# zuds-survey/zuds-pipeline

Measured on AMD Instinct MI355X. Metric: Mpix/s resample->coadd->subtract, 3072x3072 frames, higher is better.
Workload: dtype f32; 1 GPU; configs[1]+[2]: 32x 3072x3072 TPV frames/GPU, mesh background + weight rescale + Lanczos-3 resample + WEIGHTED coadd (+ AND mask coadd, int16 masks); then 1 science frame/GPU: align ref, hotpants 3x3 regions x 10x10 stamps, r=10, ko=4, subtract; frames_per_gpu=32, size=3072, mask_dtype=int16, combine=WEIGHTED, subtract=True

## Files before the change

zuds-pipeline_amd/csrc/hotpants.hip:

```cpp
#include "hp_dev.h"
#include <sched.h>
#include "chol_diag.h"

__global__ void k_hp_valid(const float* __restrict__ sci, const float* __restrict__ ref,
                           const uint8_t* __restrict__ bpm, int64_t n, float il, float iu,
                           float tl, float tu, uint8_t* __restrict__ bad,
                           const double* __restrict__ lim, double nsig) {
    int64_t p = (int64_t)blockIdx.x * blockDim.x + threadIdx.x;
    if (lim) {
        il = (float)(lim[0] - nsig * lim[1]);
        tl = (float)(lim[3] - nsig * lim[4]);
    }
    if (p >= n) return;
    float s = sci[p], t = ref[p];
    bool ok = (s == s) && (t == t) && fabsf(s) < 3e38f && fabsf(t) < 3e38f;
    ok = ok && s >= il && s <= iu && t >= tl && t <= tu;
    if (bpm) ok = ok && bpm[p] == 0;
    bad[p] = ok ? 0 : 1;
}

#define HP_ROWMAX 16384
__global__ __launch_bounds__(256) void k_hp_rowany(const uint8_t* __restrict__ in, int nx, int ny, int hw,
                                                   uint8_t* __restrict__ out) {
    extern __shared__ int ra_pre[];
// ... 2258 lines not shown
    hp_merit_body(P, G, phi, vbar, active, xsol, merit, guard, needlist);
}
__global__ __launch_bounds__(64) void k_hp_merit_b(const hp_plan P, const hp_job* __restrict__ jobs, int round) {
    const hp_job& J = jobs[blockIdx.z];
    hp_merit_body(P, J.G, J.phi, J.vbar, J.active, J.rhs, J.merit, HPJ_GUARD(J, round), J.needlist);
}

__global__ __launch_bounds__(64) void k_hp_reject_wave(const hp_plan P, const double* __restrict__ merit,
                                                       const int2* __restrict__ centres, int* __restrict__ active,
                                                       int* __restrict__ need, int* __restrict__ chg,
                                                       int* __restrict__ nrej, double* __restrict__ stats,
                                                       const int* __restrict__ guard, int* __restrict__ round_flag,
                                                       int* __restrict__ needlist, const int* __restrict__ tmo,
                                                       const hp_sig sig) {
    hp_reject_wave_body(P, merit, centres, active, need, chg, nrej, stats, guard, round_flag, needlist, tmo);
    hp_round_signal(sig, round_flag, gridDim.x);
}
__global__ __launch_bounds__(64) void k_hp_reject_wave_b(const hp_plan P, const hp_job* __restrict__ jobs, int round) {
    const hp_job& J = jobs[blockIdx.z];
    hp_reject_wave_body(P, J.merit, J.centres, J.active, J.need, J.chg, HPJ_NREJ(J), J.stats, HPJ_GUARD(J, round),
                        J.rflags + round, J.needlist);
}

__global__ void k_hp_flag(int32_t* __restrict__ mask, const float* __restrict__ img, float value, int32_t bit,
                          int64_t n, const int* __restrict__ tmo, int nreg) {
    int gaveup = 0;
    for (int r = 0; r < nreg; ++r) gaveup |= tmo[r];
    if (gaveup) return;
    int64_t p = (int64_t)blockIdx.x * blockDim.x + threadIdx.x;
    if (p >= n) return;
    if (img[p] == value) mask[p] |= bit;
}

extern "C" void zm_hp_params_default(zm_hp_params* p) {
    if (!p) return;
    memset(p, 0, sizeof(*p));
    p->tu = 5e3; p->tl = 0.0; p->iu = 5e3; p->il = 0.0;
    p->r = 10.0; p->rss = 15.0;
    p->fin = sqrt(50000.0); p->fi = 1e-30;
    p->nsx = p->nsy = 10; p->nrx = p->nry = 1;
    p->ko = 4; p->bgo = 0; p->nss = 3; p->normalize = 0;
    p->ft = 20.0; p->ks = 2.0;
    p->ngauss = 3;
    p->deg[0] = 6; p->deg[1] = 4; p->deg[2] = 2;
    p->sigma[0] = 0.7; p->sigma[1] = 1.5; p->sigma[2] = 3.0;
    p->limits_dev = nullptr; p->limits_nsigma = 10.0;
}

static int make_plan(const zm_hp_params* hp, int nx, int ny, hp_plan* P, std::vector<double>* filt,
                     std::vector<double>* basis) {
    memset(P, 0, sizeof(*P));
    P->nx = nx; P->ny = ny;
    P->hwk = (int)hp->r; P->hwss = (int)hp->rss;
    ZM_CHECK(P->hwk >= 1 && P->hwk <= HP_MAX_HWK, "zm_subtract: kernel half width int(r) = %d outside [1, %d]", P->hwk, HP_MAX_HWK);
    ZM_CHECK(P->hwss >= 1 && P->hwss <= HP_MAX_HWSS, "zm_subtract: substamp half width int(rss) = %d outside [1, %d]", P->hwss, HP_MAX_HWSS);
    P->hw = P->hwk + P->hwss;
    P->step = 2 * P->hwk + 1; P->sw = 2 * P->hwss + 1; P->pw = 2 * P->hw + 1;
    P->npix = P->sw * P->sw;
    P->npixp = (P->npix + GR_KT - 1) / GR_KT * GR_KT;
    ZM_CHECK(hp->ngauss >= 1 && hp->ngauss <= 4, "zm_subtract: ngauss %d outside [1, 4]", hp->ngauss);
    ZM_CHECK(hp->ko >= 0 && hp->ko <= 6, "zm_subtract: -ko %d outside [0, 6]", hp->ko);
    ZM_CHECK(hp->bgo >= 0 && hp->bgo <= 3, "zm_subtract: -bgo %d outside [0, 3]", hp->bgo);
    ZM_CHECK(hp->nss >= 1 && hp->nss <= HP_MAXNSS, "zm_subtract: nss %d outside [1, %d]", hp->nss, HP_MAXNSS);
    ZM_CHECK(hp->nrx >= 1 && hp->nry >= 1 && hp->nrx * hp->nry <= HP_MAXREG, "zm_subtract: bad -nrx/-nry");
    ZM_CHECK(hp->nsx >= 1 && hp->nsy >= 1 && hp->nsx * hp->nsy <= 4096, "zm_subtract: bad -nsx/-nsy");
    P->ko = hp->ko; P->bgo = hp->bgo; P->nss = hp->nss; P->normalize = hp->normalize;
// ... 288 lines not shown
    const int* h_int = reinterpret_cast<const int*>(h_sum);
    const double* h_stats = reinterpret_cast<const double*>(h_sum + sizeof(int) * HP_NIBUF);
    const double* h_x0 = h_stats + 2 * HP_MAXREG;
    int rounds = 0, retries = 0, ntimeouts = 0;
    const char* spin_env = getenv("ZM_CHOL_SPIN_LIMIT");
    hp_fit_guard fitting(&g_hp_fitting[ctx->device & 63]);
    for (int attempt = 0; attempt < 2; ++attempt) {
    const bool safe = attempt > 0;
    const int spin_limit = (!safe && spin_env) ? atoi(spin_env) : CF_SPIN_LIMIT;
    ZM_HIP(hipMemsetAsync(ibuf, 0, sizeof(int) * HP_NIBUF, st));
    ZM_TRY(hp_launch_cells(ctx, P, ref, bad, dirty, centres, active, need, ntotal));
    const hv_cfg hvc = hp_vectors_cfg(P.pw, P.sw, P.npix);
    ZM_CHECK(hvc.cw >= 8, "zm_subtract: r = %d, rss = %d: the template patch alone exceeds the LDS", P.hwk, P.hwss);
    size_t vsh = hvc.shmem;
    const int hv_gx = hvc.big ? std::min(P.ncell, 128) : P.ncell;
    double* hv_w0g = nullptr;
    if (hvc.w0_global)
        ZM_TRY(ctx->get("hp_w0g", sizeof(double) * (size_t)hv_gx * HV_SPLIT_FEW * P.npix, (void**)&hv_w0g));

    int* rflags = nullptr;
    int* h_rflags = nullptr;
    hipEvent_t* evs = nullptr;
    ZM_TRY(ctx->get("hp_rflags", sizeof(int) * 32, (void**)&rflags));
    ZM_TRY(ctx->get_pinned("hp_rflags_h", sizeof(int) * 16, (void**)&h_rflags));
    ZM_TRY(zm_get_sync_events(ctx, 3, &evs));
    ZM_HIP(hipMemsetAsync(rflags, 0, sizeof(int) * 32, st));
    if (!ctx->hp_sig_h) {
        ZM_HIP(hipHostMalloc((void**)&ctx->hp_sig_h, sizeof(unsigned long long) * 16, hipHostMallocCoherent | hipHostMallocMapped));
        memset(ctx->hp_sig_h, 0, sizeof(unsigned long long) * 16);
        ZM_HIP(hipHostGetDevicePointer((void**)&ctx->hp_sig_d, ctx->hp_sig_h, 0));
    }
    static const bool sig_off = ZM_DEVENV("ZM_HP_SIGNAL") && ZM_DEVENV("ZM_HP_SIGNAL")[0] == '0';
    const unsigned seq = ++ctx->hp_seq;
    auto enqueue_round = [&](const int rounds) -> int {
        const int* guard = rounds > 1 ? rflags + (rounds - 1) : nullptr;
        const int ncl_grid = std::min(P.ncell, 48);
        if (rounds > 1) {
            zm_scope_timer t(ctx, "hp_solve");
            int nt = zm_div_up(P.nunk, 16);
            if (P.nkp > 16)
                hipLaunchKernelGGL(k_hp_build, dim3(nt, nt, P.nreg), b256, 0, st, P, G, phi, active, chg, -1, A0, rhs0, guard);
        }
        {
            zm_scope_timer t(ctx, "hp_vectors");
            ZM_TRY(zm_hp_launch_vectors(ctx, st, P, hvc, rounds, ncl_grid, hv_gx, sci, ref, sci_rms, ref_rms, d_filt, centres, active,
                                        need, X, phi, vbar, guard, phiold, needlist, hv_w0g));
            ZM_HIP(hipGetLastError());
        }
        {
            zm_scope_timer t(ctx, "hp_gram");
            hipLaunchKernelGGL(k_hp_gram, dim3(rounds == 1 ? P.ncell : ncl_grid, GR_SPLIT), b256, 0, st, P, X, need, active, Gp, guard,
                               rounds == 1 ? nullptr : needlist);
            hipLaunchKernelGGL(k_hp_gram_sum, dim3(rounds == 1 ? P.ncell : ncl_grid), dim3(GS_THREADS), 0, st, Gp, need, active, G, guard, Gold,
                               rounds == 1 ? nullptr : needlist);
            ZM_HIP(hipGetLastError());
        }
        {
            zm_scope_timer t(ctx, "hp_solve");
            int nt = zm_div_up(P.nunk, 16);
            const char* form_env = getenv("ZM_CHOL_FORM");
            bool tp = safe || ctx->share >= 2 || fitting.shared();
            if (form_env && !strcmp(form_env, "tp")) tp = true;
            if (form_env && (!strcmp(form_env, "lat") || !strcmp(form_env, "df")) && !safe) tp = false;
            if (!ctx->hp_wg_cap) {
                int occ = 0, ncu = 0;
                ZM_HIP(hipOccupancyMaxActiveBlocksPerMultiprocessor(&occ, (const void*)k_chol_fused, 256, 0));
                ZM_HIP(hipDeviceGetAttribute(&ncu, hipDeviceAttributeMultiprocessorCount, ctx->device));
                ctx->hp_wg_cap = std::max(1, std::min(occ, 1) * (ncu - ncu / 16));
                if (ZM_DEVENV("ZM_CHOL_PROF")) fprintf(stderr, "chol: occupancy %d x %d CUs\n", occ, ncu);
            }
            const int wg_cap = ctx->hp_wg_cap / std::max(ctx->share, 1);
            const int W = std::max(2, std::min(68, wg_cap / P.nreg));
            const int nunk = P.nunk;
            static const bool want_prof = ZM_DEVENV("ZM_CHOL_PROF") && atoi(ZM_DEVENV("ZM_CHOL_PROF")) != 0;
            const bool want_df = !tp && !(form_env && !strcmp(form_env, "lat")) && 2 * P.nreg <= wg_cap && W <= 128;
            const int ndff = hp_df_nflags(P.nunk);
            unsigned* dff = nullptr;
            double* dfdg = nullptr;
            int* dftiles = nullptr;
            bool df = want_df;
            if (df) {
                constexpr int TW = 1 + 2 * DF_MAXT;
                int* htl = nullptr;
                ZM_TRY(ctx->get_pinned("hp_dftiles_h", sizeof(int) * (3 + 128 * TW), (void**)&htl));
                ZM_TRY(ctx->get("hp_dftiles", sizeof(int) * 128 * TW, (void**)&dftiles));
                constexpr int DF_MAGIC = 0x64663031;
                const bool known = htl[2] == DF_MAGIC && htl[1] == W && (htl[0] == nunk || htl[0] == -nunk - 1);
                if (!known) {
                    ZM_HIP(hipStreamSynchronize(st));
                    bool fits = true;
                    for (int wg = 0; wg < W; ++wg) {
                        int ti[DF_MAXT] = {0, 0, 0}, tj[DF_MAXT] = {0, 0, 0}, ntl = 0;
                        fits = hp_df_owner(nunk, W, wg, ti, tj, &ntl) && fits;
                        htl[3 + wg * TW] = ntl;
                        for (int k = 0; k < DF_MAXT; ++k) { htl[3 + wg * TW + 1 + 2 * k] = ti[k]; htl[3 + wg * TW + 2 + 2 * k] = tj[k]; }
                    }
                    htl[0] = fits ? nunk : -nunk - 1;
                    htl[1] = W;
                    htl[2] = DF_MAGIC;
                    if (fits) ZM_HIP(hipMemcpyAsync(dftiles, htl + 3, sizeof(int) * W * TW, hipMemcpyHostToDevice, st));
                }
                df = htl[0] == nunk;
            }
            if (df) {
                ZM_TRY(ctx->get("hp_dfflags", sizeof(unsigned) * (size_t)ndff * P.nreg, (void**)&dff));
                ZM_TRY(ctx->get("hp_dfdg", sizeof(double) * (size_t)P.nreg * zm_div_up(P.nunk, CH_NB) * CH_NB * (CH_NB + 1),
                                (void**)&dfdg));
            }
            static const bool build_scalar = ZM_DEVENV("ZM_BUILD_FORM") && !strcmp(ZM_DEVENV("ZM_BUILD_FORM"), "scalar");
            if (P.nkp <= 15 && rounds == 1 && !build_scalar)
                hipLaunchKernelGGL(k_hp_build_mfma, dim3(zm_div_up(P.nE * (P.nE + 1) / 2, 4), P.nreg), b256, 0, st, P, G, phi, active,
                                   A0, rhs0, dff, ndff);
            else if (P.nkp <= 16)
                hipLaunchKernelGGL(k_hp_build_blk, dim3(zm_div_up(P.nE * (P.nE + 1) / 2, HBB_PAIRS), 1, P.nreg), b256, 0, st, P, G, phi, active, chg,
                                   rounds == 1 ? 0 : 2, A0, rhs0, guard, dff, ndff, Gold, phiold, need);
            else
                hipLaunchKernelGGL(k_hp_build, dim3(nt, nt, P.nreg), b256, 0, st, P, G, phi, active, chg,
                                   rounds == 1 ? 0 : 1, A0, rhs0, guard, dff, ndff);
            if (!df) {
                hipLaunchKernelGGL(k_hp_diag, dim3(zm_div_up(P.nunk, 256), P.nreg), b256, 0, st, P.nunk, A0, dsc, guard);
                hipLaunchKernelGGL(k_hp_scale, dim3(zm_div_up(P.nunk, 256), P.nunk, P.nreg), b256, 0, st, P.nunk, lda,
                                   A0, rhs0, A, dsc, cbar, guard, nullptr, 0);
            }
            {
                if (tp) {
                    static const bool tp_prof = ZM_DEVENV("ZM_CHOL_PROF") && atoi(ZM_DEVENV("ZM_CHOL_PROF")) != 0;
                    long long* parg = nullptr;
                    if (tp_prof) ZM_TRY(ctx->get("hp_cprof", sizeof(long long) * 5 * P.nreg, (void**)&parg));
                    const int ldt = (P.nunk + 1 + 15) & ~15;
                    double* AT = nullptr;
                    ZM_TRY(ctx->get("hp_chol_at", sizeof(double) * (size_t)P.nreg * P.nunk * ldt, (void**)&AT));
                    {
                        zm_scope_timer tc(ctx, "hp_chol");
                        hipLaunchKernelGGL(k_chol_tp, dim3(P.nreg), dim3(CT_THREADS), 0, st, P.nunk, lda, ldt, A, AT, fail, parg, guard);
                    }
                    ZM_HIP(hipGetLastError());
                    if (tp_prof) {
                        std::vector<long long> hp((size_t)5 * P.nreg);
                        ZM_HIP(hipMemcpyAsync(hp.data(), parg, sizeof(long long) * hp.size(), hipMemcpyDeviceToHost, st));
                        ZM_HIP(hipStreamSynchronize(st));
                        static const char* nm[5] = {"init", "products", "diag", "factor", "solve"};
                        fprintf(stderr, "chol_tp wg 0:");
                        for (int k = 0; k < 5; ++k) fprintf(stderr, " %s %.1f us", nm[k], hp[k] * 0.01);
                        fprintf(stderr, "\n");
                    }
                } else {
                ZM_CHECK(2 * P.nreg <= wg_cap,
                         "zm_subtract: %d regions exceed the %d resident workgroups of this context's share (1 / %d)",
                         P.nreg, wg_cap, ctx->share);
                const int nprof = df ? 8 : 6;
                long long* parg = nullptr;
// ... 75 lines not shown
        if (sig_off) {
            ZM_HIP(hipMemcpyAsync(h_rflags + rounds, rflags + rounds, sizeof(int), hipMemcpyDeviceToHost, st));
            ZM_HIP(hipEventRecord(evs[1 + (rounds & 1)], st));
        }
        return 0;
    };
    auto wait_round = [&](int r, int* flag) -> int {
        if (sig_off) {
            ZM_HIP(hipEventSynchronize(evs[1 + (r & 1)]));
            *flag = h_rflags[r];
            return 0;
        }
        for (unsigned long spins = 1;; ++spins) {
            const unsigned long long w = __atomic_load_n(&ctx->hp_sig_h[r], __ATOMIC_ACQUIRE);
            if ((unsigned)(w >> 32) == seq && ((unsigned)w & HP_RFLAG_DONE)) {
                *flag = (int)((unsigned)w & ~HP_RFLAG_DONE);
                return 0;
            }
            if ((spins & 0x3ffff) == 0) {
                const hipError_t e = hipStreamQuery(st);
                if (e == hipSuccess) {
                    const unsigned long long w2 = __atomic_load_n(&ctx->hp_sig_h[r], __ATOMIC_ACQUIRE);
                    ZM_CHECK((unsigned)(w2 >> 32) == seq && ((unsigned)w2 & HP_RFLAG_DONE),
                             "zm_subtract: round %d finished without signalling the host", r);
                } else if (e != hipErrorNotReady) {
                    ZM_HIP(e);
                }
            }
            if (spins < 4096) __builtin_ia32_pause();
            else sched_yield();
        }
    };
    rounds = 0;
    ZM_TRY(enqueue_round(1));
    bool tmo_seen = false;
    for (int r = 1; r <= 8; ++r) {
        if (r < 8) ZM_TRY(enqueue_round(r + 1));
        int flag = 0;
        ZM_TRY(wait_round(r, &flag));
        rounds = r;
        tmo_seen = tmo_seen || (flag & HP_RFLAG_TMO);
        if ((flag & ~HP_RFLAG_TMO) == 0 || tmo_seen) break;
    }
    {
        zm_scope_timer t(ctx, "hp_apply");
        unsigned long long* smask = nullptr;
        ZM_TRY(ctx->get("hp_smask", sizeof(unsigned long long), (void**)&smask));
        hipLaunchKernelGGL(k_hp_solved, dim3(1), dim3(64), 0, st, P.nreg, P.nunk, stats, fail, tmo, rhs, smask, x0sum);
        {
            ZM_TRY(zm_hp_launch_apply(ctx, P, smask, sci, ref, sci_rms, ref_rms, outbad, d_filt, rhs, out_diff, out_rms, nmasked));
        }
    }
    if (hp->flag_mask_dev) {
        hipLaunchKernelGGL(k_hp_flag, dim3((unsigned)((np + 255) / 256)), b256, 0, st, hp->flag_mask_dev, out_diff, 1e-30f,
                           hp->flag_bit, np, tmo, P.nreg);
        ZM_HIP(hipGetLastError());
    }
    ZM_HIP(hipMemcpyAsync(h_sum, sumbuf, HP_SUMBYTES, hipMemcpyDeviceToHost, st));
    if (hp->async_info && !tmo_seen) {
        if (!ctx->hp_done) ZM_HIP(hipEventCreateWithFlags(&ctx->hp_done, hipEventDisableTiming));
        ZM_HIP(hipEventRecord(ctx->hp_done, st));
        ctx->hp_pending = true;
        ctx->hp_pend_rounds = rounds;
        ctx->hp_pend_retries = retries;
        ctx->hp_pend_nreg = P.nreg;
        ctx->hp_pend_nunk = P.nunk;
        fitting.release();
        if (info) {
            memset(info, 0, sizeof(*info));
            info->status = ZM_HP_PENDING;
            info->niter = rounds;
            info->ncoeff = P.nunk;
            info->retries = retries;
        }
        return 0;
// ... 118 lines not shown
    }
    for (int j = 0; j < njobs; ++j) {
        char* sb = base + slab * (size_t)j;
        hp_job& J = h_jobs[j];
        J.sci = jobs[j].sci; J.ref = jobs[j].ref; J.srms = jobs[j].sci_rms; J.trms = jobs[j].ref_rms;
        J.centres = (int2*)(sb + o_centres);
        J.active = (int*)(sb + o_active); J.need = (int*)(sb + o_need); J.needlist = (int*)(sb + o_needlist);
        J.chg = (int*)(sb + o_chg);
        J.ibuf = ibuf_all + (size_t)HP_NIBUF * j; J.rflags = rflags_all + 16 * (size_t)j;
        J.X = (double*)(sb + o_X); J.G = (double*)(sb + o_G); J.Gp = (double*)(sb + o_Gp); J.Gold = (double*)(sb + o_Gold);
        J.phi = (double*)(sb + o_phi); J.phiold = (double*)(sb + o_phiold); J.vbar = (double*)(sb + o_vbar);
        J.A = (double*)(sb + o_A); J.AT = (double*)(sb + o_AT); J.rhs = (double*)(sb + o_rhs);
        J.A0 = (double*)(sb + o_A0); J.rhs0 = (double*)(sb + o_rhs0); J.dsc = (double*)(sb + o_dsc);
        J.merit = (double*)(sb + o_merit); J.stats = sum_all + (size_t)3 * HP_MAXREG * j;
        J.smask = (unsigned long long*)(sb + o_smask);
    }
    ZM_HIP(hipMemcpyAsync(d_jobs, h_jobs, sizeof(hp_job) * (size_t)njobs, hipMemcpyHostToDevice, st));
    ZM_HIP(hipMemsetAsync(ibuf_all, 0, sizeof(int) * HP_NIBUF * (size_t)njobs, st));
    ZM_HIP(hipMemsetAsync(rflags_all, 0, sizeof(int) * 16 * (size_t)njobs, st));

    for (int j = 0; j < njobs; ++j) {
        char* sb = base + slab * (size_t)j;
        const hp_job& J = h_jobs[j];
        ZM_TRY(hp_launch_masks(ctx, Pj[j], jobs[j].params, jobs[j].sci, jobs[j].ref, jobs[j].bpm, (uint8_t*)(sb + o_bad), tmp8,
                               (uint8_t*)(sb + o_dirty), (uint8_t*)(sb + o_outbad)));
        ZM_TRY(hp_launch_cells(ctx, Pj[j], jobs[j].ref, (uint8_t*)(sb + o_bad), (uint8_t*)(sb + o_dirty), J.centres, J.active,
                               J.need, HPJ_NTOTAL(J)));
    }

    const size_t vsh = hp_vectors_cfg(P.pw, P.sw, P.npix).shmem;
    const dim3 b256(256);
    std::vector<int> live(njobs);
    for (int j = 0; j < njobs; ++j) live[j] = j;
    auto enqueue_round = [&](const int round) -> int {
        zm_scope_timer t(ctx, "hpb_fit");
        const hp_job* d_tab = d_jobs;
        unsigned NJ = (unsigned)njobs;
        if (round >= 3) {
            hp_job* h_tab = h_jobs + (size_t)njobs * (round - 1);
            for (size_t k = 0; k < live.size(); ++k) h_tab[k] = h_jobs[live[k]];
            NJ = (unsigned)live.size();
            if (NJ == 0) return 0;
            d_tab = d_jobs + (size_t)njobs * (round - 1);
            ZM_HIP(hipMemcpyAsync((void*)d_tab, h_tab, sizeof(hp_job) * NJ, hipMemcpyHostToDevice, st));
        }
        const int ncl_grid = std::min(P.ncell, 12);
        const unsigned gcells = round == 1 ? P.ncell : ncl_grid;
        ZM_TRY(zm_hp_launch_vectors_b(ctx, st, P, vsh, gcells, NJ, d_tab, d_filt, round));
        hipLaunchKernelGGL(k_hp_gram_b, dim3(gcells, GR_SPLIT, NJ), b256, 0, st, P, d_tab, round);
        hipLaunchKernelGGL(k_hp_gram_sum_b, dim3(gcells, 1, NJ), dim3(GS_THREADS), 0, st, d_tab, round);
        static const bool build_scalar = ZM_DEVENV("ZM_BUILD_FORM") && !strcmp(ZM_DEVENV("ZM_BUILD_FORM"), "scalar");
        if (round == 1 && !build_scalar)
            hipLaunchKernelGGL(k_hp_build_mfma_b, dim3(zm_div_up(P.nE * (P.nE + 1) / 2, 4), P.nreg, NJ), b256, 0, st, P, d_tab);
        else
            hipLaunchKernelGGL(k_hp_build_blk_b, dim3(zm_div_up(P.nE * (P.nE + 1) / 2, HBB_PAIRS), NJ, P.nreg), b256, 0, st, P, d_tab, round);
        hipLaunchKernelGGL(k_hp_diag_b, dim3(zm_div_up(P.nunk, 256), P.nreg, NJ), b256, 0, st, P.nunk, d_tab, round);
        hipLaunchKernelGGL(k_hp_scale_b, dim3(zm_div_up(P.nunk, HSB_ROWS), P.nreg * NJ), b256, 0, st, P.nunk, lda, P.nreg,
                           d_tab, round, P.ncell, P.ncellr);
        hipLaunchKernelGGL(k_chol_tp_b, dim3(P.nreg, 1, NJ), dim3(CT_THREADS), 0, st, P.nunk, lda, ldt, d_tab, round, P.ncell, P.ncellr);
        hipLaunchKernelGGL(k_chol_back_cols_b, dim3(P.nreg, 1, NJ), dim3(CBC_THREADS), 0, st, P.nunk, lda, d_tab, round, P.ncell, P.ncellr);
        hipLaunchKernelGGL(k_hp_merit_b, dim3(P.ncell, 1, NJ), dim3(64), 0, st, P, d_tab, round);
        hipLaunchKernelGGL(k_hp_reject_wave_b, dim3(P.nreg, 1, NJ), dim3(64), 0, st, P, d_tab, round);
        ZM_HIP(hipGetLastError());
        ZM_HIP(hipMemcpyAsync(h_rflags + 16 * (size_t)njobs * (round & 1), rflags_all, sizeof(int) * 16 * (size_t)njobs,
                              hipMemcpyDeviceToHost, st));
        ZM_HIP(hipEventRecord(evs[1 + (round & 1)], st));
        return 0;
    };
    auto enqueue_apply = [&](const int j) -> int {
        zm_scope_timer t(ctx, "hp_apply");
        char* sb = base + slab * (size_t)j;
        const hp_job& J = h_jobs[j];
        hipLaunchKernelGGL(k_hp_solved, dim3(1), dim3(64), 0, ctx->stream, P.nreg, P.nunk, J.stats, HPJ_FAIL(J), HPJ_TMO(J),
                           J.rhs, J.smask, J.stats + 2 * HP_MAXREG);
        ZM_TRY(zm_hp_launch_apply(ctx, Pj[j], J.smask, jobs[j].sci, jobs[j].ref, jobs[j].sci_rms, jobs[j].ref_rms,
                                  (uint8_t*)(sb + o_outbad), d_filt, J.rhs, jobs[j].out_diff, jobs[j].out_rms, HPJ_NMASKED(J)));
        if (jobs[j].params->flag_mask_dev)
            ZM_TRY(zm_mask_flag_dev(ctx, jobs[j].params->flag_mask_dev, jobs[j].out_diff, 1e-30f, jobs[j].params->flag_bit, np));
        return 0;
    };
    static const bool apply_beside = !(ZM_DEVENV("ZM_BATCH_APPLY") && !strcmp(ZM_DEVENV("ZM_BATCH_APPLY"), "after"));
// ... 139 lines not shown
```

zuds-pipeline_amd/csrc/hp_dev.h:

```cpp
#pragma once
#include <algorithm>
#include <atomic>
#include <cmath>

#include "zm_internal.h"

#define HP_MAXX 64
#define HP_MAXPOLY 28
#define HP_MAXNSS 8
#define HP_MAXREG 64
#define CF_BAR_STRIDE 32
#define HP_MAXF1 32
#define HP_RIDGE 1e-10

struct hp_plan {
    int nx, ny, hwk, hwss, hw, step, sw, npix, npixp, pw;
    int nc, nbg, nE, nX, nkp, nunk, ko, bgo;
    int nrx, nry, nsx, nsy, nss, nreg, ncellr, ncell, nf1;
    int normalize;
    double tu, tl, iu, il, ft, ks;
    float fi, fin;
    int rx0[HP_MAXREG], rx1[HP_MAXREG], ry0[HP_MAXREG], ry1[HP_MAXREG];
    int tfx[HP_MAXX], tfy[HP_MAXX], tsub0[HP_MAXX];
    double tscale[HP_MAXX];
// ... 13 lines not shown
template <int NW>
__device__ inline double block_sum_waves(double v, double* red) {
    v = wave_sum_d(v);
    __syncthreads();
    if ((threadIdx.x & 63) == 0) red[threadIdx.x >> 6] = v;
    __syncthreads();
    double t[NW];
#pragma unroll
    for (int w = 0; w < NW; ++w) t[w] = red[w];
#pragma unroll
    for (int step = 1; step < NW; step *= 2)
#pragma unroll
        for (int w = 0; w + step < NW; w += 2 * step) t[w] += t[w + step];
    return t[0];
}

__device__ inline double block_sum256(double v, double* red) {
    v = wave_sum_d(v);
    __syncthreads();
    if ((threadIdx.x & 63) == 0) red[threadIdx.x >> 6] = v;
    __syncthreads();
    return (red[0] + red[1]) + (red[2] + red[3]);
}

__device__ inline double ipowd(double x, int n) {
    double r = 1.0;
    for (int k = 0; k < n; ++k) r *= x;
    return r;
}

#define HV_R 8
#define HV_SPLIT_ALL 5
#define HV_SPLIT_FEW 16

#define HV_THREADS 512
#define HP_MAX_HWK 20
#define HP_MAX_HWSS 60
struct hv_cfg { bool big; bool w0_global; int cw; size_t shmem; };
static inline hv_cfg hp_vectors_cfg(int pw, int sw, int npix) {
    const size_t lim = 160 * 1024, patch = sizeof(float) * (size_t)pw * (pw + 8) + 16;
    const size_t fast = sizeof(double) * ((size_t)(pw + 8) * sw + npix + 8) + patch;
    if (fast <= lim) return {false, false, sw, fast};
    const size_t full = sizeof(double) * ((size_t)(pw + 8) * sw + 8) + patch;
    if (full <= lim) return {true, true, sw, full};
    if (patch + sizeof(double) * 8 + sizeof(double) * (size_t)(pw + 8) * 8 > lim) return {true, true, 0, 0};
    int cw = (int)((lim - patch - sizeof(double) * 8) / (sizeof(double) * (size_t)(pw + 8)));
    cw &= ~7;
    return {true, true, cw, sizeof(double) * ((size_t)(pw + 8) * cw + 8) + patch};
}

struct hp_job {
    const float *sci, *ref, *srms, *trms;
    int2* centres;
    int *active, *need, *needlist, *chg, *ibuf, *rflags;
    double *X, *G, *Gp, *Gold, *phi, *phiold, *vbar, *A, *AT, *rhs, *A0, *rhs0, *dsc, *merit, *stats;
    unsigned long long* smask;
};
#define HPJ_NREJ(J) ((J).ibuf)
#define HPJ_NTOTAL(J) ((J).ibuf + HP_MAXREG)
#define HPJ_FAIL(J) ((J).ibuf + 2 * HP_MAXREG)
#define HPJ_NMASKED(J) ((J).ibuf + 3 * HP_MAXREG)
#define HPJ_TMO(J) ((J).ibuf + 3 * HP_MAXREG + 4)
#define HPJ_GUARD(J, round) ((round) > 1 ? (J).rflags + ((round) - 1) : nullptr)
#define HPJ_REGION_IDLE(J, round, reg, ncell, ncellr) ((round) > 1 && (J).chg[(ncell) + (reg) * ((ncellr) + 1)] == 0)

int zm_hp_launch_vectors(zm_ctx* ctx, hipStream_t st, const hp_plan& P, const hv_cfg& hvc, int rounds, int ncl_grid, int hv_gx,
                         const float* sci, const float* ref, const float* sci_rms, const float* ref_rms, const double* filt,
                         const int2* centres, const int* active, const int* need, double* X, double* phi, double* vbar,
                         const int* guard, double* phiold, const int* needlist, double* hv_w0g);
int zm_hp_launch_vectors_b(zm_ctx* ctx, hipStream_t st, const hp_plan& P, size_t vsh, unsigned gcells, unsigned njobs,
                           const hp_job* d_tab, const double* filt, int round);
int zm_hp_launch_apply(zm_ctx* ctx, const hp_plan& P, const unsigned long long* solved_mask, const float* sci,
                       const float* ref, const float* srms, const float* trms, const uint8_t* outbad,
                       const double* filt, const double* xsol, float* diff, float* noise, int* nmasked);
```

zuds-pipeline_amd/csrc/hp_vectors.hip:

```cpp
#include "hp_dev.h"

template <int HWK, bool BIG = false>
static __device__ __forceinline__ void hp_vectors_body(const hp_plan& P, const float* __restrict__ sci,
                                                    const float* __restrict__ ref,
                                                    const float* __restrict__ srms,
                                                    const float* __restrict__ trms,
                                                    const double* __restrict__ filt,
                                                    const int2* __restrict__ centres,
                                                    const int* __restrict__ active,
                                                    const int* __restrict__ need,
                                                    double* __restrict__ X,
                                                    double* __restrict__ phi,
                                                    double* __restrict__ vbar, const int* __restrict__ guard,
                                                    double* __restrict__ phiold, const int* __restrict__ list,
                                                    int special, int cwarg = 0, double* __restrict__ w0g = nullptr) {
    if (guard && *guard == 0) return;
    extern __shared__ double hp_smem[];
    constexpr int STEP = 2 * HWK + 1;
    constexpr int WIN = HV_R + 2 * HWK;
    const int tid = threadIdx.x;
    const int part = blockIdx.y, nparts = gridDim.y;
    const int ncl = list ? list[0] : (BIG ? P.ncell : (int)gridDim.x);
#pragma unroll 1
    for (int ci = blockIdx.x; ci < ncl; ci += gridDim.x) {
    const int cell = list ? list[1 + ci] : ci;
    __syncthreads();
    if (!need[cell]) continue;
    const int act = active[cell];
    if (act < 0) continue;
    const int2 cc = centres[cell * P.nss + act];
    const int r = cell / P.ncellr;
    const int pw = P.pw, sw = P.sw, hwss = P.hwss;
    const bool only_special = special && part == 0;
    const int fpart = special ? part - 1 : part, fparts = special ? nparts - 1 : nparts;
    const int pp = pw + HV_R;
    const int cw = BIG ? cwarg : P.sw;
    double* xp = hp_smem;
    double* w0 = (BIG && w0g) ? w0g + ((size_t)blockIdx.y * gridDim.x + blockIdx.x) * (size_t)P.npix
                              : xp + (size_t)(pw + HV_R) * cw;
    double* red = (BIG && w0g) ? xp + (size_t)(pw + HV_R) * cw : w0 + P.npix;
    float* patch = reinterpret_cast<float*>(red + 8);
    for (int k0 = tid; !only_special && k0 < pw * pw; k0 += HV_THREADS * 10) {
        float t[10];
#pragma unroll
        for (int u = 0; u < 10; ++u) {
            const int k = k0 + HV_THREADS * u;
            const int yy = k / pw, xx = k - yy * pw;
            t[u] = (k < pw * pw) ? ref[(size_t)(cc.y - P.hw + yy) * P.nx + (cc.x - P.hw + xx)] : 0.f;
// ... 30 lines not shown
#pragma unroll
        for (int u = 0; u < 5; ++u) {
            int k = k0 + 256 * u;
            asm volatile("" : "+v"(k));
            if (k < P.npix) {
                const int i = k / sw, j = k - i * sw;
                const int x = cc.x - hwss + j, y = cc.y - hwss + i;
                Xc[(size_t)P.nE * P.npixp + k] = (double)ts[u];
                const double a = ta[u], b = tb[u];
                vs += a * a + b * b;
                const double xf = (x - xc) / hx, yf = (y - yc) / hy;
                for (int q = 0; q < P.nbg; ++q)
                    Xc[(size_t)(P.nc + q) * P.npixp + k] = ipowd(xf, P.bpi[q]) * ipowd(yf, P.bpj[q]);
            } else if (k < P.npixp) {
                for (int q = 0; q < P.nX; ++q) Xc[(size_t)q * P.npixp + k] = 0.0;
            }
        }
    }
    vs = block_sum_waves<HV_THREADS / 64>(vs, red);
    if (tid == 0 && part == 0) {
        vbar[cell] = vs / P.npix;
        double fx = (cc.x - xc) / hx, fy = (cc.y - yc) / hy;
        if (phiold) {
#pragma clang loop vectorize(disable) interleave(disable) unroll(disable)
            for (int p = 0; p < P.nkp; ++p) phiold[(size_t)cell * P.nkp + p] = phi[(size_t)cell * P.nkp + p];
        }
#pragma clang loop vectorize(disable) interleave(disable) unroll(disable)
        for (int p = 0; p < P.nkp; ++p)
            phi[(size_t)cell * P.nkp + p] = ipowd(fx, P.kpi[p]) * ipowd(fy, P.kpj[p]);
    }
    __syncthreads();
    if (only_special) continue;
    const int nstrip = (sw + HV_R - 1) / HV_R;
    int fidx = 0;
    for (int f = 0; f < P.nf1; ++f) {
        const int tn0 = P.tf0[f], tn1 = tn0 + P.tfn[f];
        if (tn1 == tn0) continue;
        const bool mine = (fidx % fparts) == fpart;
        ++fidx;
        const bool for_w0 = (P.tfx[0] == f);
        if (!mine && !for_w0) continue;
        const double* fxv = filt + f * STEP;
        const int nchunks = BIG ? (sw + cw - 1) / cw : 1;
        for (int ch = 0; ch < nchunks; ++ch) {
        const int c0 = BIG ? ch * cw : 0;
        const int cwe = BIG ? min(cw, sw - c0) : sw;
        const int nstripc = BIG ? (cwe + HV_R - 1) / HV_R : nstrip;
        for (int e = tid; e < pw * nstripc; e += HV_THREADS) {
            const int yy = e / nstripc, jl0 = (e - yy * nstripc) * HV_R, j0 = c0 + jl0;
            const float* pr = patch + yy * pp + j0;
            double wv[WIN];
#pragma unroll
            for (int k = 0; k < WIN; ++k) wv[k] = (double)pr[k];
            double acc[HV_R];
#pragma unroll
            for (int q = 0; q < HV_R; ++q) acc[q] = 0.0;
#pragma unroll
            for (int m = 0; m < STEP; ++m) {
                const double cf = fxv[2 * HWK - m];
#pragma unroll
                for (int q = 0; q < HV_R; ++q) acc[q] += cf * wv[q + m];
            }
#pragma unroll
            for (int q = 0; q < HV_R; ++q)
                if (j0 + q < sw) xp[yy * cw + jl0 + q] = acc[q];
        }
        __syncthreads();
        for (int n = tn0; n < tn1; ++n) {
            if (!mine && n != 0) continue;
            const double* fyv = filt + P.tfy[n] * STEP;
            const double sc = P.tscale[n];
            const bool sub0 = n != 0 && P.tsub0[n] != 0;
            for (int e = tid; e < cwe * nstrip; e += HV_THREADS) {
// ... 33 lines not shown
            if (n == 0) __syncthreads();
        }
        __syncthreads();
        }
    }
    }
}

template <int HWK>
__global__ __launch_bounds__(HV_THREADS) void k_hp_vectors(const hp_plan P, const float* __restrict__ sci,
                                                    const float* __restrict__ ref, const float* __restrict__ srms,
                                                    const float* __restrict__ trms, const double* __restrict__ filt,
                                                    const int2* __restrict__ centres, const int* __restrict__ active,
                                                    const int* __restrict__ need, double* __restrict__ X,
                                                    double* __restrict__ phi, double* __restrict__ vbar,
                                                    const int* __restrict__ guard, double* __restrict__ phiold,
                                                    const int* __restrict__ list, int special) {
    hp_vectors_body<HWK>(P, sci, ref, srms, trms, filt, centres, active, need, X, phi, vbar, guard, phiold, list, special);
}
template <int HWK>
__global__ __launch_bounds__(HV_THREADS) void k_hp_vectors_big(const hp_plan P, const float* __restrict__ sci,
                                                    const float* __restrict__ ref, const float* __restrict__ srms,
                                                    const float* __restrict__ trms, const double* __restrict__ filt,
                                                    const int2* __restrict__ centres, const int* __restrict__ active,
                                                    const int* __restrict__ need, double* __restrict__ X,
                                                    double* __restrict__ phi, double* __restrict__ vbar,
                                                    const int* __restrict__ guard, double* __restrict__ phiold,
                                                    const int* __restrict__ list, int special, int cw, double* __restrict__ w0g) {
    hp_vectors_body<HWK, true>(P, sci, ref, srms, trms, filt, centres, active, need, X, phi, vbar, guard, phiold, list, special,
                               cw, w0g);
}
template <int HWK>
__global__ __launch_bounds__(HV_THREADS, (HWK <= 11 ? 4 : 2)) void k_hp_vectors_b(const hp_plan P, const hp_job* __restrict__ jobs,
                                                      const double* __restrict__ filt, int round) {
    const hp_job& J = jobs[blockIdx.z];
    hp_vectors_body<HWK>(P, J.sci, J.ref, J.srms, J.trms, filt, J.centres, J.active, J.need, J.X, J.phi, J.vbar,
                         HPJ_GUARD(J, round), J.phiold, round > 1 ? J.needlist : nullptr, round > 1 ? 1 : 0);
}


int zm_hp_launch_vectors(zm_ctx* ctx, hipStream_t st, const hp_plan& P, const hv_cfg& hvc, int rounds, int ncl_grid, int hv_gx,
                         const float* sci, const float* ref, const float* sci_rms, const float* ref_rms, const double* d_filt,
                         const int2* centres, const int* active, const int* need, double* X, double* phi, double* vbar,
                         const int* guard, double* phiold, const int* needlist, double* hv_w0g) {
    const size_t vsh = hvc.shmem;
    const dim3 grid_s(rounds == 1 ? P.ncell : ncl_grid, rounds == 1 ? HV_SPLIT_ALL : HV_SPLIT_FEW);
    const dim3 grid_b(rounds == 1 ? hv_gx : std::min(ncl_grid, hv_gx), rounds == 1 ? HV_SPLIT_ALL : HV_SPLIT_FEW);
    const int* list = rounds == 1 ? nullptr : needlist;
    const int special = rounds == 1 ? 0 : 1;
    if (hvc.big) {
#define C(H) case H: \
    ZM_HIP(hipFuncSetAttribute((const void*)k_hp_vectors_big<H>, hipFuncAttributeMaxDynamicSharedMemorySize, (int)vsh)); \
    hipLaunchKernelGGL(k_hp_vectors_big<H>, grid_b, dim3(HV_THREADS), vsh, st, P, sci, ref, sci_rms, ref_rms, d_filt, \
                       centres, active, need, X, phi, vbar, guard, phiold, list, special, hvc.cw, hv_w0g); break;
        switch (P.hwk) {
            C(1) C(2) C(3) C(4) C(5) C(6) C(7) C(8) C(9) C(10) C(11) C(12) C(13) C(14) C(15) C(16) C(17) C(18) C(19) C(20)
            default: zm_set_error("zm_subtract: unsupported kernel half width %d", P.hwk); return 2;
        }
#undef C
    } else {
#define C(H) case H: \
    ZM_HIP(hipFuncSetAttribute((const void*)k_hp_vectors<H>, hipFuncAttributeMaxDynamicSharedMemorySize, (int)vsh)); \
    hipLaunchKernelGGL(k_hp_vectors<H>, grid_s, dim3(HV_THREADS), vsh, st, P, sci, ref, sci_rms, ref_rms, d_filt, \
                       centres, active, need, X, phi, vbar, guard, phiold, list, special); break;
        switch (P.hwk) {
            C(1) C(2) C(3) C(4) C(5) C(6) C(7) C(8) C(9) C(10) C(11) C(12) C(13) C(14) C(15) C(16) C(17) C(18) C(19) C(20)
            default: zm_set_error("zm_subtract: unsupported kernel half width %d", P.hwk); return 2;
        }
#undef C
    }
    ZM_HIP(hipGetLastError());
    return 0;
}

int zm_hp_launch_vectors_b(zm_ctx* ctx, hipStream_t st, const hp_plan& P, size_t vsh, unsigned gcells, unsigned NJ,
                           const hp_job* d_tab, const double* d_filt, int round) {
#define C(H) case H: \
    ZM_HIP(hipFuncSetAttribute((const void*)k_hp_vectors_b<H>, hipFuncAttributeMaxDynamicSharedMemorySize, (int)vsh)); \
    hipLaunchKernelGGL(k_hp_vectors_b<H>, dim3(gcells, round == 1 ? HV_SPLIT_ALL : HV_SPLIT_FEW, NJ), dim3(HV_THREADS), vsh, st, \
                       P, d_tab, d_filt, round); break;
    switch (P.hwk) {
        C(1) C(2) C(3) C(4) C(5) C(6) C(7) C(8) C(9) C(10) C(11) C(12) C(13) C(14) C(15)
        default: zm_set_error("zm_subtract: unsupported kernel half width %d", P.hwk); return 2;
    }
#undef C
    return 0;
}
```

Before: 48930 Mpix/s.

## Split hotpants vector work by basis term and defer solve until round flag

Adds a per-term partitioning of the convolution-vector kernel for later fitting rounds, so each y-block handles a fixed small group of basis terms instead of filters taken round-robin. The grid height is sized from the term count. The round loop is also split into rebuild and solve phases, and by default the next round's solve is enqueued only after the host has read the current round's flag. This avoids speculative Cholesky work, at the cost of less host/GPU overlap. An env var restores the old form.

Result: no change. 49040 Mpix/s (median of 6 runs) (+0.2%).

```diff
diff --git a/zuds-pipeline_amd/csrc/hotpants.hip b/zuds-pipeline_amd/csrc/hotpants.hip
--- a/zuds-pipeline_amd/csrc/hotpants.hip
+++ b/zuds-pipeline_amd/csrc/hotpants.hip
@@ -2314,6 +2314,11 @@
     if (img[p] == value) mask[p] |= bit;
 }
 
+static bool hp_fit_form_r6() {
+    const char* e = getenv("ZM_FIT_FORM");
+    return e && !strcmp(e, "r6");
+}
+
 extern "C" void zm_hp_params_default(zm_hp_params* p) {
     if (!p) return;
     memset(p, 0, sizeof(*p));
@@ -2668,7 +2673,10 @@
     }
     static const bool sig_off = ZM_DEVENV("ZM_HP_SIGNAL") && ZM_DEVENV("ZM_HP_SIGNAL")[0] == '0';
     const unsigned seq = ++ctx->hp_seq;
-    auto enqueue_round = [&](const int rounds) -> int {
+    const bool fit_new = !hp_fit_form_r6();
+    struct hp_round_form { bool tp, df; int wg_cap, W, ndff; unsigned* dff; double* dfdg; int* dftiles; };
+    hp_round_form form{};
+    auto enqueue_rebuild = [&](const int rounds) -> int {
         const int* guard = rounds > 1 ? rflags + (rounds - 1) : nullptr;
         const int ncl_grid = std::min(P.ncell, 48);
         if (rounds > 1) {
@@ -2680,7 +2688,7 @@
         {
             zm_scope_timer t(ctx, "hp_vectors");
             ZM_TRY(zm_hp_launch_vectors(ctx, st, P, hvc, rounds, ncl_grid, hv_gx, sci, ref, sci_rms, ref_rms, d_filt, centres, active,
-                                        need, X, phi, vbar, guard, phiold, needlist, hv_w0g));
+                                        need, X, phi, vbar, guard, phiold, needlist, hv_w0g, fit_new));
             ZM_HIP(hipGetLastError());
         }
         {
@@ -2708,7 +2716,6 @@
             const int wg_cap = ctx->hp_wg_cap / std::max(ctx->share, 1);
             const int W = std::max(2, std::min(68, wg_cap / P.nreg));
             const int nunk = P.nunk;
-            static const bool want_prof = ZM_DEVENV("ZM_CHOL_PROF") && atoi(ZM_DEVENV("ZM_CHOL_PROF")) != 0;
             const bool want_df = !tp && !(form_env && !strcmp(form_env, "lat")) && 2 * P.nreg <= wg_cap && W <= 128;
             const int ndff = hp_df_nflags(P.nunk);
             unsigned* dff = nullptr;
@@ -2753,6 +2760,20 @@
             else
                 hipLaunchKernelGGL(k_hp_build, dim3(nt, nt, P.nreg), b256, 0, st, P, G, phi, active, chg,
                                    rounds == 1 ? 0 : 1, A0, rhs0, guard, dff, ndff);
+            form = hp_round_form{tp, df, wg_cap, W, ndff, dff, dfdg, dftiles};
+        }
+        return 0;
+    };
+    auto enqueue_solve = [&](const int rounds) -> int {
+        const int* guard = rounds > 1 ? rflags + (rounds - 1) : nullptr;
+        {
+            zm_scope_timer t(ctx, "hp_solve");
+            const bool tp = form.tp, df = form.df;
+            const int wg_cap = form.wg_cap, W = form.W, nunk = P.nunk;
+            unsigned* const dff = form.dff;
+            double* const dfdg = form.dfdg;
+            int* const dftiles = form.dftiles;
+            static const bool want_prof = ZM_DEVENV("ZM_CHOL_PROF") && atoi(ZM_DEVENV("ZM_CHOL_PROF")) != 0;
             if (!df) {
                 hipLaunchKernelGGL(k_hp_diag, dim3(zm_div_up(P.nunk, 256), P.nreg), b256, 0, st, P.nunk, A0, dsc, guard);
                 hipLaunchKernelGGL(k_hp_scale, dim3(zm_div_up(P.nunk, 256), P.nunk, P.nreg), b256, 0, st, P.nunk, lda,
@@ -2894,15 +2915,18 @@
         }
     };
     rounds = 0;
-    ZM_TRY(enqueue_round(1));
+    ZM_TRY(enqueue_rebuild(1));
+    ZM_TRY(enqueue_solve(1));
     bool tmo_seen = false;
     for (int r = 1; r <= 8; ++r) {
-        if (r < 8) ZM_TRY(enqueue_round(r + 1));
+        if (r < 8) ZM_TRY(enqueue_rebuild(r + 1));
+        if (r < 8 && !fit_new) ZM_TRY(enqueue_solve(r + 1));
         int flag = 0;
         ZM_TRY(wait_round(r, &flag));
         rounds = r;
         tmo_seen = tmo_seen || (flag & HP_RFLAG_TMO);
         if ((flag & ~HP_RFLAG_TMO) == 0 || tmo_seen) break;
+        if (r < 8 && fit_new) ZM_TRY(enqueue_solve(r + 1));
     }
     {
         zm_scope_timer t(ctx, "hp_apply");
@@ -3087,6 +3111,7 @@
     const dim3 b256(256);
     std::vector<int> live(njobs);
     for (int j = 0; j < njobs; ++j) live[j] = j;
+    const bool fit_new = !hp_fit_form_r6();
     auto enqueue_round = [&](const int round) -> int {
         zm_scope_timer t(ctx, "hpb_fit");
         const hp_job* d_tab = d_jobs;
@@ -3101,7 +3126,7 @@
         }
         const int ncl_grid = std::min(P.ncell, 12);
         const unsigned gcells = round == 1 ? P.ncell : ncl_grid;
-        ZM_TRY(zm_hp_launch_vectors_b(ctx, st, P, vsh, gcells, NJ, d_tab, d_filt, round));
+        ZM_TRY(zm_hp_launch_vectors_b(ctx, st, P, vsh, gcells, NJ, d_tab, d_filt, round, fit_new));
         hipLaunchKernelGGL(k_hp_gram_b, dim3(gcells, GR_SPLIT, NJ), b256, 0, st, P, d_tab, round);
         hipLaunchKernelGGL(k_hp_gram_sum_b, dim3(gcells, 1, NJ), dim3(GS_THREADS), 0, st, d_tab, round);
         static const bool build_scalar = ZM_DEVENV("ZM_BUILD_FORM") && !strcmp(ZM_DEVENV("ZM_BUILD_FORM"), "scalar");
diff --git a/zuds-pipeline_amd/csrc/hp_dev.h b/zuds-pipeline_amd/csrc/hp_dev.h
--- a/zuds-pipeline_amd/csrc/hp_dev.h
+++ b/zuds-pipeline_amd/csrc/hp_dev.h
@@ -69,6 +69,8 @@
 #define HV_R 8
 #define HV_SPLIT_ALL 5
 #define HV_SPLIT_FEW 16
+#define HV_TERMS_PER_PART 2
+static inline int hp_vectors_term_parts(int nc) { return 1 + (nc + HV_TERMS_PER_PART - 1) / HV_TERMS_PER_PART; }
 
 #define HV_THREADS 512
 #define HP_MAX_HWK 20
@@ -104,9 +106,9 @@
 int zm_hp_launch_vectors(zm_ctx* ctx, hipStream_t st, const hp_plan& P, const hv_cfg& hvc, int rounds, int ncl_grid, int hv_gx,
                          const float* sci, const float* ref, const float* sci_rms, const float* ref_rms, const double* filt,
                          const int2* centres, const int* active, const int* need, double* X, double* phi, double* vbar,
-                         const int* guard, double* phiold, const int* needlist, double* hv_w0g);
+                         const int* guard, double* phiold, const int* needlist, double* hv_w0g, bool byterm);
 int zm_hp_launch_vectors_b(zm_ctx* ctx, hipStream_t st, const hp_plan& P, size_t vsh, unsigned gcells, unsigned njobs,
-                           const hp_job* d_tab, const double* filt, int round);
+                           const hp_job* d_tab, const double* filt, int round, bool byterm);
 int zm_hp_launch_apply(zm_ctx* ctx, const hp_plan& P, const unsigned long long* solved_mask, const float* sci,
                        const float* ref, const float* srms, const float* trms, const uint8_t* outbad,
                        const double* filt, const double* xsol, float* diff, float* noise, int* nmasked);
diff --git a/zuds-pipeline_amd/csrc/hp_vectors.hip b/zuds-pipeline_amd/csrc/hp_vectors.hip
--- a/zuds-pipeline_amd/csrc/hp_vectors.hip
+++ b/zuds-pipeline_amd/csrc/hp_vectors.hip
@@ -14,6 +14,7 @@
                                                     double* __restrict__ vbar, const int* __restrict__ guard,
                                                     double* __restrict__ phiold, const int* __restrict__ list,
                                                     int special, int cwarg = 0, double* __restrict__ w0g = nullptr) {
+    const bool byterm = !BIG && special == 2;
     if (guard && *guard == 0) return;
     extern __shared__ double hp_smem[];
     constexpr int STEP = 2 * HWK + 1;
@@ -110,13 +111,34 @@
     __syncthreads();
     if (only_special) continue;
     const int nstrip = (sw + HV_R - 1) / HV_R;
+    const int bt0 = fpart * HV_TERMS_PER_PART, bt1 = min(P.nc, bt0 + HV_TERMS_PER_PART);
+    bool bt_w0 = false;
+    for (int n = bt0; byterm && n < bt1; ++n) bt_w0 = bt_w0 || (n != 0 && P.tsub0[n] != 0);
+    int bt_next = bt0;
     int fidx = 0;
-    for (int f = 0; f < P.nf1; ++f) {
-        const int tn0 = P.tf0[f], tn1 = tn0 + P.tfn[f];
-        if (tn1 == tn0) continue;
-        const bool mine = (fidx % fparts) == fpart;
-        ++fidx;
-        const bool for_w0 = (P.tfx[0] == f);
+    const int nsteps = byterm ? 1 + HV_TERMS_PER_PART : P.nf1;
+    for (int it = 0; it < nsteps; ++it) {
+        int f, tn0, tn1;
+        bool mine, for_w0;
+        if (byterm) {
+            if (it == 0) {
+                if (!bt_w0 || bt0 == 0) continue;
+                f = P.tfx[0]; tn0 = 0; tn1 = 1; mine = false; for_w0 = true;
+            } else {
+                if (bt_next >= bt1) continue;
+                tn0 = bt_next; f = P.tfx[tn0]; tn1 = tn0 + 1;
+                while (tn1 < bt1 && P.tfx[tn1] == f) ++tn1;
+                bt_next = tn1;
+                mine = true; for_w0 = (tn0 == 0);
+            }
+        } else {
+            f = it;
+            tn0 = P.tf0[f]; tn1 = tn0 + P.tfn[f];
+            if (tn1 == tn0) continue;
+            mine = (fidx % fparts) == fpart;
+            ++fidx;
+            for_w0 = (P.tfx[0] == f);
+        }
         if (!mine && !for_w0) continue;
         const double* fxv = filt + f * STEP;
         const int nchunks = BIG ? (sw + cw - 1) / cw : 1;
@@ -216,22 +238,23 @@
 }
 template <int HWK>
 __global__ __launch_bounds__(HV_THREADS, (HWK <= 11 ? 4 : 2)) void k_hp_vectors_b(const hp_plan P, const hp_job* __restrict__ jobs,
-                                                      const double* __restrict__ filt, int round) {
+                                                      const double* __restrict__ filt, int round, int special) {
     const hp_job& J = jobs[blockIdx.z];
     hp_vectors_body<HWK>(P, J.sci, J.ref, J.srms, J.trms, filt, J.centres, J.active, J.need, J.X, J.phi, J.vbar,
-                         HPJ_GUARD(J, round), J.phiold, round > 1 ? J.needlist : nullptr, round > 1 ? 1 : 0);
+                         HPJ_GUARD(J, round), J.phiold, round > 1 ? J.needlist : nullptr, special);
 }
 
 
 int zm_hp_launch_vectors(zm_ctx* ctx, hipStream_t st, const hp_plan& P, const hv_cfg& hvc, int rounds, int ncl_grid, int hv_gx,
                          const float* sci, const float* ref, const float* sci_rms, const float* ref_rms, const double* d_filt,
                          const int2* centres, const int* active, const int* need, double* X, double* phi, double* vbar,
-                         const int* guard, double* phiold, const int* needlist, double* hv_w0g) {
+                         const int* guard, double* phiold, const int* needlist, double* hv_w0g, bool byterm) {
     const size_t vsh = hvc.shmem;
-    const dim3 grid_s(rounds == 1 ? P.ncell : ncl_grid, rounds == 1 ? HV_SPLIT_ALL : HV_SPLIT_FEW);
+    const dim3 grid_s(rounds == 1 ? P.ncell : ncl_grid,
+                      rounds == 1 ? HV_SPLIT_ALL : (byterm ? hp_vectors_term_parts(P.nc) : HV_SPLIT_FEW));
     const dim3 grid_b(rounds == 1 ? hv_gx : std::min(ncl_grid, hv_gx), rounds == 1 ? HV_SPLIT_ALL : HV_SPLIT_FEW);
     const int* list = rounds == 1 ? nullptr : needlist;
-    const int special = rounds == 1 ? 0 : 1;
+    const int special = rounds == 1 ? 0 : (byterm && !hvc.big ? 2 : 1);
     if (hvc.big) {
 #define C(H) case H: \
     ZM_HIP(hipFuncSetAttribute((const void*)k_hp_vectors_big<H>, hipFuncAttributeMaxDynamicSharedMemorySize, (int)vsh)); \
@@ -258,11 +281,13 @@
 }
 
 int zm_hp_launch_vectors_b(zm_ctx* ctx, hipStream_t st, const hp_plan& P, size_t vsh, unsigned gcells, unsigned NJ,
-                           const hp_job* d_tab, const double* d_filt, int round) {
+                           const hp_job* d_tab, const double* d_filt, int round, bool byterm) {
+    const unsigned gy = round == 1 ? HV_SPLIT_ALL : (byterm ? hp_vectors_term_parts(P.nc) : HV_SPLIT_FEW);
+    const int special = round == 1 ? 0 : (byterm ? 2 : 1);
 #define C(H) case H: \
     ZM_HIP(hipFuncSetAttribute((const void*)k_hp_vectors_b<H>, hipFuncAttributeMaxDynamicSharedMemorySize, (int)vsh)); \
-    hipLaunchKernelGGL(k_hp_vectors_b<H>, dim3(gcells, round == 1 ? HV_SPLIT_ALL : HV_SPLIT_FEW, NJ), dim3(HV_THREADS), vsh, st, \
-                       P, d_tab, d_filt, round); break;
+    hipLaunchKernelGGL(k_hp_vectors_b<H>, dim3(gcells, gy, NJ), dim3(HV_THREADS), vsh, st, \
+                       P, d_tab, d_filt, round, special); break;
     switch (P.hwk) {
         C(1) C(2) C(3) C(4) C(5) C(6) C(7) C(8) C(9) C(10) C(11) C(12) C(13) C(14) C(15)
         default: zm_set_error("zm_subtract: unsupported kernel half width %d", P.hwk); return 2;
```
